# klasmodin/quflow

Measured on AMD Instinct MI355X. Metric: isospectral timesteps/sec at N=1024 (1 GPU) + ensemble steps/sec at 1/2/4/8 GPUs, higher is better.
Workload: dtype f64

## Files before the change

include/quflow_hip.h:

```cpp
#ifndef QUFLOW_HIP_H
#define QUFLOW_HIP_H

#ifdef __cplusplus
extern "C" {
#endif

#define QF_OK 0
#define QF_ERR_INVALID 1
#define QF_ERR_NO_DEVICE 2
#define QF_ERR_HIP 3
#define QF_ERR_STATE 4
#define QF_ERR_CALLBACK 5
#define QF_ERR_UNSUPPORTED 6
#define QF_ERR_NONFINITE 7
#define QF_ERR_NOCONVERGE 8

#define QF_VERSION 100

typedef struct qf_ctx qf_ctx;

int qf_version(void);
const char *qf_last_error(void);
int qf_device_count(void);

// ... 156 lines not shown
#define QF_BUF_W 0
#define QF_BUF_DW 1
#define QF_BUF_WHALF 2
#define QF_BUF_PHALF 3
#define QF_BUF_PW 4
int qf_download_buffer(qf_ctx *ctx, int which, void *host);
int qf_debug_guard_check(long long *allocations, long long *damaged, char *first, int n);
int qf_debug_modulus(qf_ctx *ctx, int n, const double *er_host, const double *ei_host, double *out_modulus_host,
                     double *out_sqrt_host);
int qf_zgemm(qf_ctx *ctx, const void *A_host, const void *B_host, void *C_host);
int qf_commutator(qf_ctx *ctx, const void *W_host, const void *P_host, void *C_host, int skewherm);
int qf_zgemm_i8(qf_ctx *ctx, const void *A_host, const void *B_host, void *C_host);
int qf_fixedpoint_products(qf_ctx *ctx, const void *Phalf_host, const void *Whalf_host, const void *W_host,
                           const void *dW_old_host, int variant, void *dW_new_host, void *Whalf_new_host,
                           double *rowsum_host);

int qf_c64_laplacian_table(qf_ctx *ctx, int bc, float *lap_host);
int qf_c64_solve_poisson(qf_ctx *ctx, const void *W_host, void *P_host, int skewh);
int qf_c64_solve_tridiagonal(qf_ctx *ctx, const float *lap_host, const void *W_host, void *P_host, int skewh);
int qf_c64_laplace(qf_ctx *ctx, const void *P_host, void *W_host);
int qf_c64_upload_W(qf_ctx *ctx, const void *W_host);
int qf_c64_download_W(qf_ctx *ctx, void *W_host);
int qf_c64_isomp(qf_ctx *ctx, double dt, int steps, double tol, int minit, int maxit, int compsum, int reinitialize,
                 qf_isomp_stats *stats_out);
int qf_c64_isomp_continue(qf_ctx *ctx, double dt, int steps, double tol, int minit, int maxit, int compsum, int reinitialize,
                          qf_isomp_stats *stats_out);
int qf_c64_diagnostics(qf_ctx *ctx, double *energy_euler, double *enstrophy);
int qf_cgemm(qf_ctx *ctx, const void *A_host, const void *B_host, void *C_host);
int qf_c64_fixedpoint_products(qf_ctx *ctx, const void *Phalf_host, const void *Whalf_host, const void *W_host,
                               const void *dW_old_host, void *dW_new_host, void *Whalf_new_host, double *rowsum_host);
// ... 16 lines not shown
```

quflow_amd/_lib.py:

```python
import ctypes
import os

_HERE = os.path.dirname(os.path.abspath(__file__))
LIB_PATH = os.environ.get("QUFLOW_HIP_LIB") or os.path.join(_HERE, "libquflow_hip.so")

QF_OK = 0
QF_ERR_NONFINITE = 7
QF_ERR_NOCONVERGE = 8
ERR_NAMES = {1: "QF_ERR_INVALID", 2: "QF_ERR_NO_DEVICE", 3: "QF_ERR_HIP", 4: "QF_ERR_STATE", 5: "QF_ERR_CALLBACK",
             6: "QF_ERR_UNSUPPORTED", 7: "QF_ERR_NONFINITE", 8: "QF_ERR_NOCONVERGE"}

KERNEL_IDS = {"poisson": 0, "gemm1": 1, "gemm2": 2, "norm": 3, "update": 4, "slice": 5}
ERK_METHODS = {"euler": 0, "heun": 1, "rk4": 2}
BUFFER_IDS = {"W": 0, "dW": 1, "Whalf": 2, "Phalf": 3, "PW": 4}


class QuflowHipError(RuntimeError):
    pass


HAMILTONIAN_CB = ctypes.CFUNCTYPE(ctypes.c_int, ctypes.c_void_p, ctypes.c_void_p, ctypes.c_void_p, ctypes.c_double)
FORCING_CB = ctypes.CFUNCTYPE(ctypes.c_int, ctypes.c_void_p, ctypes.c_void_p, ctypes.c_void_p, ctypes.c_void_p, ctypes.c_double)
STRANG_CB = ctypes.CFUNCTYPE(ctypes.c_int, ctypes.c_void_p, ctypes.c_double, ctypes.c_void_p)
CALLBACK_CB = ctypes.CFUNCTYPE(ctypes.c_int, ctypes.c_void_p, ctypes.c_void_p, ctypes.c_void_p)
# ... 134 lines not shown
    "qf_profile_reset": (ctypes.c_int, [_vp]),
    "qf_profile_read": (ctypes.c_int, [_vp, ctypes.c_int, ctypes.POINTER(ctypes.c_longlong), _dp]),
    "qf_plan_describe": (ctypes.c_int, [_vp, ctypes.c_char_p, ctypes.c_int]),
    "qf_device_info": (ctypes.c_int, [ctypes.c_int, ctypes.c_char_p, ctypes.c_int]),
    "qf_debug_modulus": (ctypes.c_int, [_vp, ctypes.c_int, _dp, _dp, _dp, _dp]),
    "qf_profile_stride": (ctypes.c_int, [_vp, ctypes.c_int]),
    "qf_profile_seen": (ctypes.c_int, [_vp, ctypes.c_int, ctypes.POINTER(ctypes.c_longlong)]),
    "qf_timer_start": (ctypes.c_int, [_vp]),
    "qf_timer_stop": (ctypes.c_int, [_vp, _dp]),
    "qf_download_buffer": (ctypes.c_int, [_vp, ctypes.c_int, _vp]),
    "qf_debug_guard_check": (ctypes.c_int, [ctypes.POINTER(ctypes.c_longlong), ctypes.POINTER(ctypes.c_longlong), ctypes.c_char_p, ctypes.c_int]),
    "qf_zgemm": (ctypes.c_int, [_vp, _vp, _vp, _vp]),
    "qf_commutator": (ctypes.c_int, [_vp, _vp, _vp, _vp, ctypes.c_int]),
    "qf_zgemm_i8": (ctypes.c_int, [_vp, _vp, _vp, _vp]),
    "qf_fixedpoint_products": (ctypes.c_int, [_vp, _vp, _vp, _vp, _vp, ctypes.c_int, _vp, _vp, _vp]),
    "qf_c64_laplacian_table": (ctypes.c_int, [_vp, ctypes.c_int, _vp]),
    "qf_c64_solve_poisson": (ctypes.c_int, [_vp, _vp, _vp, ctypes.c_int]),
    "qf_c64_laplace": (ctypes.c_int, [_vp, _vp, _vp]),
    "qf_c64_solve_tridiagonal": (ctypes.c_int, [_vp, _vp, _vp, _vp, ctypes.c_int]),
    "qf_c64_upload_W": (ctypes.c_int, [_vp, _vp]),
    "qf_c64_download_W": (ctypes.c_int, [_vp, _vp]),
    "qf_c64_isomp": (ctypes.c_int, [_vp, ctypes.c_double, ctypes.c_int, ctypes.c_double, ctypes.c_int,
                                    ctypes.c_int, ctypes.c_int, ctypes.c_int, ctypes.POINTER(IsompStats)]),
    "qf_c64_isomp_continue": (ctypes.c_int, [_vp, ctypes.c_double, ctypes.c_int, ctypes.c_double, ctypes.c_int,
                                             ctypes.c_int, ctypes.c_int, ctypes.c_int, ctypes.POINTER(IsompStats)]),
    "qf_c64_diagnostics": (ctypes.c_int, [_vp, _dp, _dp]),
    "qf_cgemm": (ctypes.c_int, [_vp, _vp, _vp, _vp]),
    "qf_c64_fixedpoint_products": (ctypes.c_int, [_vp, _vp, _vp, _vp, _vp, _vp, _vp, _vp]),
    "qf_c64_fixedpoint_products_tri": (ctypes.c_int, [_vp, _vp, _vp, _vp, _vp, _vp, _vp, _vp]),
}
# ... 50 lines not shown
```

quflow_amd/csrc/api_context.hip:

```cpp
#include <cmath>
#include <cstdarg>
#include <cstdio>
#include <cstdlib>
#include <cstring>
#include <limits>
#include <chrono>

#include "qf_api.h"

static thread_local char g_err[512] = "";

void qf_set_error(const char *fmt, ...)
{
    va_list ap;
    va_start(ap, fmt);
    vsnprintf(g_err, sizeof(g_err), fmt, ap);
    va_end(ap);
}

extern "C" {

int qf_version(void) { return QF_VERSION; }

int qf_device_info(int device, char *buf, int n)
// ... 101 lines not shown
        if (g[0] == 'i' && strstr(g, "x65")) ctx->oz_digits2 = 5;
        if (g[0] == 'i' && strchr(g, 'h')) ctx->gemm_i8_hybrid = true;
        if (g[0] == 'i' && strchr(g, 'f') && !ctx->gemm_i8_hybrid) ctx->gemm_i8_first = true;
        if (g[0] == 'a') {
            ctx->gemm_i8_allowed = true;
            ctx->oz_digits = 6;
            ctx->oz_digits2 = 5;
            ctx->gemm_i8_min_n = 1024;
        }
    }
    if (const char *g = getenv("QUFLOW_HIP_GEMM2")) ctx->gemm_tri_allowed = !(g[0] == 'f');
    if (const char *g = getenv("QUFLOW_HIP_FUSED")) ctx->fused_allowed = !(g[0] == '0');
    if (const char *g = getenv("QUFLOW_HIP_I8_MIN_N")) ctx->gemm_i8_min_n = atoi(g);
    if (const char *g = getenv("QUFLOW_HIP_TRI_MIN_N")) ctx->gemm_tri_min_n = atoi(g);
    if (const char *g = getenv("QUFLOW_HIP_DEFER")) ctx->defer_allowed = !(g[0] == '0');
    if (getenv("QUFLOW_HIP_DEBUG"))
        if (const char *g = getenv("QUFLOW_HIP_DEBUG_DROP_FLAG")) ctx->debug_drop = atoi(g);
    if (const char *g = getenv("QUFLOW_HIP_FACTOR_CACHE_MB")) ctx->factor_budget_bytes = (size_t)(atoi(g) > 0 ? atoi(g) : 1) << 20;
    const size_t NN = (size_t)N * N;
    const size_t mbytes = NN * sizeof(cplx);
    int rc = QF_OK;
    auto fail = [&](int code) {
        qf_ctx_destroy(ctx);
        return code;
    };
#define QF_CREATE_HIP(call)                                                                   \
    do {                                                                                      \
        hipError_t _e = (call);                                                               \
        if (_e != hipSuccess) {                                                               \
            qf_set_error("%s failed: %s", #call, hipGetErrorString(_e));                     \
// ... 45 lines not shown
    *out = ctx;
    return QF_OK;
}

int qf_ctx_destroy(qf_ctx *ctx)
{
    if (!ctx) return QF_OK;
    (void)hipSetDevice(ctx->device);
    if (ctx->stream) (void)hipStreamSynchronize(ctx->stream);
    void *ptrs[] = {ctx->W, ctx->dW[0], ctx->dW[1], ctx->Whalf, ctx->Phalf, ctx->PW, ctx->kahan_c, ctx->stage,
                    ctx->lap, ctx->lap_user, ctx->poisson.tab, ctx->ham.tab, ctx->ham_offset, ctx->forcing_f0, ctx->stoch.basis, ctx->stoch.omega,
                    ctx->stoch.stage, ctx->stoch.sigma, ctx->rowpart, ctx->rowsum,
                    ctx->t32_partial, ctx->t32_arrive, ctx->W2, ctx->Whalf2, ctx->ns_inv, ctx->ns_tmp, ctx->multi_rowpart, ctx->scalars, ctx->sk_partial, ctx->sk_flags, ctx->basis, ctx->sh_stage, ctx->sh_omega, ctx->slab};
    for (void *p : ptrs)
        if (p) (void)hipFree(p);
    void *sht[] = {ctx->sht.omega, ctx->sht.tab, ctx->sht.col, ctx->sht.At, ctx->sht.tw, ctx->sht.f, ctx->sht.H, ctx->sht.Q};
    for (void *p : sht)
        if (p) (void)hipFree(p);
    void *eigh[] = {ctx->eigh.H, ctx->eigh.G, ctx->eigh.V, ctx->eigh.ray, ctx->eigh.sig, ctx->eigh.perm, ctx->eigh.word};
    for (void *p : eigh)
        if (p) (void)hipFree(p);
    void *geom[] = {ctx->geom.R[0], ctx->geom.R[1], ctx->geom.grad};
    for (void *p : geom)
        if (p) (void)hipFree(p);
    for (hipEvent_t e : ctx->geom.ev)
        if (e) (void)hipEventDestroy(e);
    for (cplx *p : ctx->multi)
        if (p) (void)hipFree(p);
    for (cplx *p : ctx->stack)
        if (p) (void)hipFree(p);
// ... 221 lines not shown
```

quflow_amd/csrc/api_isomp.hip:

```cpp
#include <cmath>
#include <cstdarg>
#include <cstdio>
#include <cstdlib>
#include <cstring>
#include <limits>
#include <chrono>
#include <type_traits>
#include <utility>

#include "qf_api.h"

namespace {

#ifndef QF_RUN_AHEAD
#define QF_RUN_AHEAD 3
#endif

template <class S> constexpr bool is_c64 = std::is_same<S, qf_c64>::value;

template <class S> S *ws(qf_ctx *ctx)
{
    if constexpr (is_c64<S>) return ctx->c64;
    else return ctx;
}
// ... 910 lines not shown
            return QF_ERR_INVALID;
        }
        QF_TRY(tri32_alloc(ctx));
    }
    const int N = ctx->N;
    const size_t bytes = (size_t)N * N * sizeof(cplx);
    QF_HIP(hipMemcpyAsync(ctx->Phalf, Phalf_host, bytes, hipMemcpyHostToDevice, ctx->stream));
    QF_HIP(hipMemcpyAsync(ctx->Whalf, Whalf_host, bytes, hipMemcpyHostToDevice, ctx->stream));
    QF_HIP(hipMemcpyAsync(ctx->stage, W_host, bytes, hipMemcpyHostToDevice, ctx->stream));
    QF_HIP(hipMemcpyAsync(ctx->dW[0], dW_old_host, bytes, hipMemcpyHostToDevice, ctx->stream));
    QF_TRY(qf_launch_zgemm(ctx, ctx->Phalf, ctx->Whalf, ctx->PW, nullptr));
    qf_epilogue ep = epilogue_of(ctx, false);
    ep.W = ctx->stage;
    const bool saved = ctx->gemm_tri, saved32 = ctx->gemm_tri32;
    const int s_min = ctx->sk_min_units, s_epi = ctx->sk_epi_units, s_so = ctx->tri32_split, s_sd = ctx->tri32_split_diag;
    ctx->gemm_tri = (variant == 1);
    ctx->gemm_tri32 = (variant == 2);
    if (variant == 1) {
        if ((variant_arg >> 8) & 0xff) ctx->sk_min_units = (variant_arg >> 8) & 0xff;
        if ((variant_arg >> 16) & 0xff) ctx->sk_epi_units = ((variant_arg >> 16) & 0xff) - 64;
    } else if (variant == 2) {
        const int so = (variant_arg >> 8) & 15, sd = (variant_arg >> 12) & 15;
        if (so == 1 || so == 2 || so == 4) ctx->tri32_split = so;
        if (sd == 1 || sd == 2 || sd == 4) ctx->tri32_split_diag = sd;
    }
    int rc = qf_launch_zgemm(ctx, ctx->PW, ctx->Phalf, nullptr, &ep);
    ctx->gemm_tri = saved;
    ctx->gemm_tri32 = saved32;
    ctx->sk_min_units = s_min;
    ctx->sk_epi_units = s_epi;
    ctx->tri32_split = s_so;
    ctx->tri32_split_diag = s_sd;
    QF_TRY(rc);
    QF_TRY(qf_launch_sum_rowpart(ctx, ctx->rowpart, variant == 1 ? ctx->N / 64 : variant == 2 ? (ctx->N + 31) / 32 : ctx->rowpart_tiles, ctx->rowsum));
    QF_HIP(hipMemcpyAsync(dW_new_host, ctx->dW[1], bytes, hipMemcpyDeviceToHost, ctx->stream));
    QF_HIP(hipMemcpyAsync(Whalf_new_host, ctx->Whalf, bytes, hipMemcpyDeviceToHost, ctx->stream));
    QF_HIP(hipMemcpyAsync(rowsum_host, ctx->rowsum, (size_t)N * sizeof(double), hipMemcpyDeviceToHost, ctx->stream));
    QF_HIP(hipStreamSynchronize(ctx->stream));
    return QF_OK;
}


int qf_oz_alloc(qf_ctx *ctx)
{
    for (int q = 0; q < 4; ++q) {
// ... 43 lines not shown
```

quflow_amd/csrc/qf_internal.h:

```cpp
#pragma once

#include <hip/hip_runtime.h>

#include <atomic>
#include <cstdarg>
#include <cstdio>
#include <map>
#include <mutex>
#include <string>
#include <vector>

#include "../../include/quflow_hip.h"

typedef double2 cplx;

hipError_t qf_guard_malloc(void **p, size_t bytes);
hipError_t qf_guard_free(void *p);
#define hipMalloc(p, n) qf_guard_malloc((void **)(p), (n))
#define hipFree(p) qf_guard_free((void *)(p))

void qf_set_error(const char *fmt, ...);
struct qf_ctx;
inline void qf_plan_note(qf_ctx *ctx, unsigned long long key, const char *fmt, ...) __attribute__((format(printf, 3, 4)));

#define QF_HIP(call)                                                                   \
// ... 349 lines not shown
    int gemm_tri_min_n = 960;
    bool gemm_tri32 = false;
    int tri32_split = 2, tri32_split_diag = 1;
    cplx *t32_partial = nullptr;
    unsigned *t32_arrive = nullptr;
    bool defer_allowed = true;
    bool defer = false;
    int num_cus = 0;
    cplx *sk_partial = nullptr;
    unsigned *sk_flags = nullptr;
    int sk_slots = 0;
    unsigned sk_epoch = 0;
    int sk_epi_units = 0;
    int sk_epi_units_fused = 2;
    int sk_min_units = 8;
    int debug_drop = 0;
    bool needs_reset = false;

    qf_c64 *c64 = nullptr;

    int profile_mask = 0;
    std::vector<qf_event_pair> events_busy;
    std::vector<qf_event_pair> events_free;
    int profile_stride = 1;
    struct plan_slot {
        unsigned long long key = 0;
        char text[384] = {0};
    } plan[QF_KERNEL_COUNT];
    int plan_role = -1;
    long long prof_seen[QF_KERNEL_COUNT] = {0};
// ... 67 lines not shown
    qf_host_record *rec = nullptr;
    int debug_drop = 0;
};
struct qf_streamk {
    cplx *partial = nullptr;
    unsigned *flags = nullptr;
    unsigned epoch = 0;
    int *fault = nullptr;
    unsigned *ticket = nullptr;
    int n_tiles = 0;
    qf_dev_state *state_rw = nullptr;
    qf_host_record *rec = nullptr;
    unsigned spin_limit = 1u << 22;
    int debug_drop = 0;
    int slots = 0;
};
struct qf_tri32 {
    cplx *partial = nullptr;
    unsigned *arrive = nullptr;
    int split = 1;
    int split_diag = 1;
    unsigned *ticket = nullptr;
    int n_tiles = 0;
    qf_dev_state *state_rw = nullptr;
    qf_host_record *rec = nullptr;
    int debug_drop = 0;
    int deferred = 0;
};
int qf_gemm_tiles_n(int N);
int qf_launch_zgemm_tri32(qf_ctx *ctx, const cplx *A, const cplx *B, const qf_epilogue *ep, qf_guard guard = qf_guard());
int qf_launch_zgemm_tri(qf_ctx *ctx, const cplx *A, const cplx *B, const qf_epilogue *ep, qf_guard guard = qf_guard());
int qf_launch_zgemm(qf_ctx *ctx, const cplx *A, const cplx *B, cplx *C, const qf_epilogue *ep,
                    qf_guard guard = qf_guard());

int qf_launch_basis(qf_ctx *ctx, double *basis_dev);
__host__ __device__ inline long long qf_slab_prefix(int N, int Nmax, int m)
{
    const long long a = m, n = N, k = Nmax;
    return a * n * k - (n + k) * (a * (a - 1) / 2) + (a - 1) * a * (2 * a - 1) / 6;
}
int qf_slab_plan(int N, int Nmax, long long slab_bytes, std::vector<int> &first, long long *max_bytes);
int qf_launch_shr2mat(qf_ctx *ctx, int Nmax, const double *omega_dev, cplx *W_dev);
int qf_launch_band_basis(qf_ctx *ctx, int Nmax, double *band_dev);
int qf_launch_band_shr2mat(qf_ctx *ctx, int Nmax, const double *band_dev, const double *omega_dev, cplx *stage, cplx *W_dev);
int qf_launch_mat2shr(qf_ctx *ctx, int Nmax, const cplx *W_dev, double *omega_dev);
int qf_launch_shc2mat(qf_ctx *ctx, const double *omega_dev, cplx *W_dev);
// ... 73 lines not shown
```

quflow_amd/csrc/zgemm.hip:

```cpp
#include "qf_internal.h"
#include "qf_step_end.h"

#include <cstring>

typedef double v4d __attribute__((ext_vector_type(4)));

#ifdef QF_STAMP
__device__ unsigned long long *qf_stamp_buf = nullptr;
#define QF_STAMP_SLOTS 80
#ifdef QF_STAMP_LIGHT
#define QF_STAMP_AT(slot_)
#define QF_STAMP_PH(kt_, ph_)
__device__ unsigned long long *qf_phase_buf = nullptr;
#else
#define QF_STAMP_AT(slot_)                                                              \
    if (qf_stamp_buf && lane == 0 && (slot_) < QF_STAMP_SLOTS)                          \
        qf_stamp_buf[((size_t)blockIdx.x * (T / 64) + wave) * QF_STAMP_SLOTS + (slot_)] = __builtin_amdgcn_s_memtime();
__device__ unsigned long long *qf_phase_buf = nullptr;
#define QF_STAMP_PH(kt_, ph_)                                                           \
    if (qf_phase_buf && tid == 0 && (kt_) >= 20 && (kt_) < 28)                          \
        qf_phase_buf[((size_t)blockIdx.x * 8 + ((kt_) - 20)) * 5 + (ph_)] = __builtin_amdgcn_s_memtime();
#endif
__device__ unsigned long long *qf_tri_buf = nullptr;
#define QF_TRI_STAMP(seg_, k_)                                                          \
// ... 592 lines not shown
            if (tid == 0) {
                unsigned old = 0u;
                if (!((ep.debug_drop & 2) && lid == 0)) old = __hip_atomic_fetch_add(ep.ticket, 1u, __ATOMIC_RELAXED, __HIP_MEMORY_SCOPE_AGENT);
                *last_flag = (old == (unsigned)(ep.n_tiles - 1)) ? 1u : 0u;
            }
            __syncthreads();
            if (*last_flag != 0u)
                qf_fused_step_end(N, tiles_n, ep.rowpart, ep.ticket, ep.state_rw, ep.rec, guard.iter, tid, rs + WN * BM + 2);
        }
    }
    QF_STAMP_AT(KT + 2)
}

constexpr size_t TRI_SMEM_BYTES = 2 * 64 * 65 * sizeof(cplx) + 4 * 64 * sizeof(double) + 64;

__global__ __launch_bounds__(256) void k_zgemm_tri(int N, int nt, int U, int E, const cplx *__restrict__ A,
                                                    const cplx *__restrict__ B, qf_epilogue ep, qf_guard guard,
                                                    qf_streamk sk)
{
    constexpr int BM = 64, BN = 64, WM = 2, WN = 2;
    constexpr bool EPI = true, EXACT = true, FAST = true;
    using SM = tile_smem<BM, BN, true>;
    constexpr int T = WM * WN * 64;
    constexpr int WTM = BM / WM, WTN = BN / WN;
    constexpr int MT = WTM / 16, NT = WTN / 16;
    constexpr int A_STRIDE = SM::A_STRIDE, B_STRIDE = SM::B_STRIDE;
    constexpr int A_PER = (BM * BK) / T, B_PER = (BN * BK) / T;
    constexpr int A_ROWS_PER = T / BK, B_ROWS_PER = T / BN;
    constexpr int A3_STRIDE = SM::A3_STRIDE, B3_STRIDE = SM::B3_STRIDE;
    constexpr int TS = BN + 1;
    constexpr int TT_BYTES = BM * TS * (int)sizeof(cplx);
    static_assert((size_t)2 * TT_BYTES + (WN * BM + WM * BN) * sizeof(double) + 16 <= TRI_SMEM_BYTES, "epilogue scratch exceeds the LDS request");
    static_assert(TRI_SMEM_BYTES >= SM::main_bytes, "K-loop buffers exceed the LDS request");
    typedef unsigned v4u __attribute__((ext_vector_type(4)));
    constexpr int SG_MFMA = 0x008, SG_VMEM_RD = 0x020, SG_DS_WR = 0x200;

    extern __shared__ __attribute__((aligned(16))) unsigned char smem_raw[];

    const int tid = threadIdx.x;
    const int lane = tid & 63, wave = tid >> 6;
    const int wm = wave / WN, wn = wave % WN;
    const int r16_c = lane & 15, q4_c = lane >> 4;
    const int G = gridDim.x;
    const int c = xcd_remap(blockIdx.x, G);
    const int KTN = N / BK;
    const int S = KTN + E;
    int u = (int)((long long)c * U / G);
    const int u_end = (int)((long long)(c + 1) * U / G);
    const cplx zero = make_double2(0.0, 0.0);

    const unsigned char *lds_fa[2] = {
        smem_raw + (size_t)(q4_c * A_STRIDE + wm * WTM + (r16_c ^ q4_c)) * sizeof(cplx),
        smem_raw + (size_t)(q4_c * A_STRIDE + wm * WTM + (r16_c ^ q4_c ^ 4)) * sizeof(cplx)};
    const unsigned char *lds_fb = smem_raw + SM::B_OFFSET + (size_t)(q4_c * B_STRIDE + wn * WTN + r16_c) * sizeof(cplx);
    unsigned char *lds_sa = smem_raw + (size_t)((tid % BK) * A_STRIDE + ((tid / BK) ^ (tid % BK & 7))) * sizeof(cplx);
    const unsigned char *lds_fa3[2] = {
        smem_raw + SM::A3_OFFSET + (size_t)(q4_c * A3_STRIDE + wm * WTM + 2 * (r16_c ^ q4_c)) * sizeof(double),
        smem_raw + SM::A3_OFFSET + (size_t)(q4_c * A3_STRIDE + wm * WTM + 2 * (r16_c ^ q4_c ^ 4)) * sizeof(double)};
    const unsigned char *lds_fb3 = smem_raw + SM::B3_OFFSET + (size_t)(q4_c * B3_STRIDE + wn * WTN + 2 * r16_c) * sizeof(double);
    unsigned char *lds_sa3 = smem_raw + SM::A3_OFFSET + (size_t)((tid % BK) * A3_STRIDE + 2 * ((tid / BK) ^ (tid % BK & 7))) * sizeof(double);
    const int b_jA = ((tid % 32) / 16) * 32 + (tid % 16);
    unsigned char *lds_sb3 = smem_raw + SM::B3_OFFSET + (size_t)((tid / 32) * B3_STRIDE + 32 * ((tid % 32) / 16) + 2 * (tid % 16)) * sizeof(double);
    unsigned char *lds_sb = smem_raw + SM::B_OFFSET + (size_t)((tid / 32) * B_STRIDE + b_jA) * sizeof(cplx);
// ... 6 lines not shown
    const unsigned p_voff = (unsigned)(tid * sizeof(cplx));
    const unsigned char *a_row = nullptr, *b_col = nullptr;
    const size_t a_pass = 0, b_pass = 0, b_ktile = 0;
    const unsigned a_voff = 0, b_voff = 0;
    const int kt_off = 0;
    const int i0 = 0, j0 = 0;

    cplx e_c[MT][NT][4], e_t[MT][NT][4], e_w[MT][NT][4], e_old[MT][NT][4];
    v4d accR[MT][NT], accI[MT][NT], accS[MT][NT];
    cplx ra[2][A_PER], rb[2][B_PER];
    cplx fa[2][MT], fb[2][NT];
    double fas[2][MT], fbs[2][NT];
#pragma unroll
    for (int r = 0; r < A_PER; ++r) ra[1][r] = rb[1][r] = zero;

#define QF_TRI_KOF(p_) ((p_) <= 0 ? 0 : ((p_) <= E + 1 ? 1 : ((p_) - E > KTN ? KTN : (int)((p_) - E))))
#define QF_TRI_NEXT(u_, found_, t_, k0_, KT_, tm_, tn_)                                \
    {                                                                                  \
        found_ = false;                                                                \
        while (!(found_) && (u_) < u_end) {                                            \
            t_ = (int)((u_) / S);                                                      \
            const int pa_ = (u_) - (t_) * S;                                           \
            int pb_ = u_end - (t_) * S;                                                \
            if (pb_ > S) pb_ = S;                                                      \
            const int klo_ = QF_TRI_KOF(pa_), khi_ = QF_TRI_KOF(pb_);                  \
            u_ = (t_) * S + pb_;                                                       \
            if (klo_ < khi_) {                                                         \
                found_ = true;                                                         \
                k0_ = klo_;                                                            \
                KT_ = khi_ - klo_;                                                     \
                int rem_ = (t_);                                                       \
                tm_ = 0;                                                               \
                while (rem_ >= nt - (tm_)) { rem_ -= nt - (tm_); ++(tm_); }            \
                tn_ = (tm_) + rem_;                                                    \
            }                                                                          \
        }                                                                              \
    }
#define QF_TRI_START_LOADS(k0_, KT_, tm_, tn_)                                         \
    {                                                                                  \
        const int kt_of_segment_ = (KT_);                                              \
        fa_soff0 = (unsigned)(((size_t)(tm_) * BM * N + (size_t)(k0_) * BK) * sizeof(cplx)); \
        fb_soff0 = (unsigned)(((size_t)(k0_) * BK * N + (size_t)(tn_) * BN) * sizeof(cplx)); \
        {                                                                              \
            const int KT = kt_of_segment_;        \
            QF_LOAD_TILE(0, 0)                                                         \
            if (KT > 1) { QF_LOAD_TILE(1, 1) }                                         \
        }                                                                              \
    }
    int seg = 0;
    (void)seg;
// ... 87 lines not shown
                QF_EPI_COMM
            }
            QF_EPI_FETCH(e_w, ep_W, false)
            QF_EPI_FETCH(e_old, ep_dW_old, false)
            double tre[MT][NT][4], tim[MT][NT][4];
#pragma unroll
            for (int mi = 0; mi < MT; ++mi)
#pragma unroll
                for (int ni = 0; ni < NT; ++ni)
#pragma unroll
                    for (int reg = 0; reg < 4; ++reg) {
                        tre[mi][ni][reg] = accR[mi][ni][reg] - accI[mi][ni][reg];
                        tim[mi][ni][reg] = (accS[mi][ni][reg] - accR[mi][ni][reg]) - accI[mi][ni][reg];
                    }
            if (KT < KTN) {
                const int tile_org = t * S, tile_end = tile_org + S;
                const int c_first = c + 1;
                int c_last = c;
                while (c_last + 1 < G && (int)((long long)(c_last + 1) * U / G) < tile_end) ++c_last;
#define QF_TRI_HAS_PIECE(c2_)                                                          \
    (QF_TRI_KOF((int)((long long)(c2_) * U / G) - tile_org) <                          \
     QF_TRI_KOF(((int)(((long long)(c2_) + 1) * U / G) < tile_end ? (int)(((long long)(c2_) + 1) * U / G) : tile_end) - tile_org))
                for (int c2 = c_last; c2 >= c_first; --c2) {
                    const int slot2 = c2;
                    if (!QF_TRI_HAS_PIECE(c2)) continue;
                    if (tid == 0) {
                        unsigned spins = 0;
                        while (__hip_atomic_load(sk.flags + slot2, __ATOMIC_RELAXED, __HIP_MEMORY_SCOPE_AGENT) != sk.epoch) {
                            __builtin_amdgcn_s_sleep(QF_POLL_SLEEP);
                            if (++spins > sk.spin_limit) {
                                *sk.fault = 1;
                                break;
                            }
                        }
                    }
                    asm volatile("s_barrier" ::: "memory");
                    const unsigned soff = (unsigned)((size_t)slot2 * (BM * BN) * sizeof(cplx));
// ... 133 lines not shown
            }
        }
        QF_TRI_STAMP(seg, 3)
        ++seg;
        have = have_next;
        t = n_t;
        k0 = n_k0;
        KT = n_KT;
        tm = n_tm;
        tn = n_tn;
        asm volatile("s_waitcnt lgkmcnt(0)\n\ts_barrier" ::: "memory");
    }
    if (run_finale)
        qf_fused_step_end(N, nt, ep.rowpart, sk.ticket, sk.state_rw, sk.rec, guard.iter, tid, reinterpret_cast<double *>(smem_raw));
#undef QF_TRI_NEXT
#undef QF_TRI_KOF
#undef QF_TRI_HAS_PIECE
#undef QF_TRI_START_LOADS
}

template <bool EXACT>
__global__ __launch_bounds__(256) void k_zgemm_tri32(int N, int nt, const cplx *__restrict__ A, const cplx *__restrict__ B,
                                                      qf_epilogue ep, qf_guard guard, qf_tri32 sx)
{
    if (!qf_guard_iter(guard)) return;
    constexpr int BM = 32, BN = 32, WM = 2, WN = 2;
    constexpr bool EPI = true, FAST = false;
    using SM = tile_smem<BM, BN, false>;
    constexpr int T = WM * WN * 64;
    constexpr int WTM = BM / WM, WTN = BN / WN;
    constexpr int MT = WTM / 16, NT = WTN / 16;
// ... 360 lines not shown
        if (exact) return launch2<BM, BN, WM, WN, true, true>(ctx, A, B, C, *ep, guard);
        return launch2<BM, BN, WM, WN, true, false>(ctx, A, B, C, *ep, guard);
    }
    if (exact) return launch2<BM, BN, WM, WN, false, true>(ctx, A, B, C, none, guard);
    return launch2<BM, BN, WM, WN, false, false>(ctx, A, B, C, none, guard);
}

}

int qf_gemm_tiles_n(int N)
{
    gemm_cfg c = pick_gemm(N);
    return (N + c.BN - 1) / c.BN;
}

int qf_launch_zgemm_tri(qf_ctx *ctx, const cplx *A, const cplx *B, const qf_epilogue *ep, qf_guard guard)
{
    const int N = ctx->N;
    if (!ep || N % 64 != 0 || !ctx->sk_partial || ctx->num_cus < 1) {
        qf_set_error("qf_launch_zgemm_tri: not available for this context (N=%d)", N);
        return QF_ERR_STATE;
    }
    static qf_smem_attr attr;
    QF_TRY(qf_smem_attr_set(attr, (const void *)k_zgemm_tri, ctx->device, TRI_SMEM_BYTES));
    const int nt = N / 64;
    int E = ep->fused ? ctx->sk_epi_units_fused : ctx->sk_epi_units;
    if (E < -8) E = -8;
    const long long units = (long long)nt * (nt + 1) / 2 * (N / BK + E);
    if (units > 0x7fffffffLL) {
        qf_set_error("qf_launch_zgemm_tri: N=%d is too large for the stream-K partition", N);
        return QF_ERR_INVALID;
    }
    long long grid_ll = units / (ctx->sk_min_units > 0 ? ctx->sk_min_units : 1);
    if (grid_ll > ctx->num_cus) grid_ll = ctx->num_cus;
    if (grid_ll < 1) grid_ll = 1;
    const int grid = (int)grid_ll;
    qf_streamk sk;
    const int slots = ctx->sk_slots > 0 ? ctx->sk_slots : ctx->num_cus;
    sk.slots = slots;
    sk.partial = ctx->sk_partial;
    sk.flags = ctx->sk_flags;
    sk.epoch = ++ctx->sk_epoch;
    sk.fault = &ctx->host_rec->fault;
    sk.ticket = ctx->sk_flags + slots;
    sk.n_tiles = nt * (nt + 1) / 2;
    sk.state_rw = ctx->state;
    sk.rec = ctx->host_rec;
    if (ctx->debug_drop == 1 || (ctx->debug_drop == 2 && ep->fused)) {
        sk.debug_drop = ctx->debug_drop;
        sk.spin_limit = 1u << 14;
        ctx->debug_drop = 0;
    }
    qf_plan_note(ctx, 0x2000000ull | (unsigned long long)(grid << 8 | (E & 0x3f) << 1 | (ep->fused ? 1 : 0)),
                 "{\"kernel\": \"k_zgemm_tri\", \"arithmetic\": \"fp64 3M, v_mfma_f64_16x16x4_f64\", \"tile\": [64, 64], \"tiles\": %d, "
                 "\"tile_share\": %.6f, \"workgroups\": %d, \"threads\": 256, \"partition\": \"stream-K over (tile, K-tile) units, "
                 "contiguous ranges, epilogue weight E = %d K-tiles\", \"step_end\": \"%s\"}",
                 sk.n_tiles, (double)sk.n_tiles / ((double)nt * nt), grid, E, ep->fused ? "fused (last finisher decides)" : "two-kernel");
    hipLaunchKernelGGL(k_zgemm_tri, dim3(grid), dim3(256), TRI_SMEM_BYTES, ctx->stream, N, nt, (int)units, E, A, B, *ep, guard, sk);
    QF_HIP(hipGetLastError());
    return QF_OK;
}

int qf_launch_zgemm_tri32(qf_ctx *ctx, const cplx *A, const cplx *B, const qf_epilogue *ep, qf_guard guard)
{
    const int N = ctx->N;
    if (!ep || N < 64 || !ctx->t32_partial || !ctx->t32_arrive) {
        qf_set_error("qf_launch_zgemm_tri32: not available for this context (N=%d)", N);
        return QF_ERR_STATE;
    }
    const int nt = (N + 31) / 32;
    qf_tri32 sx;
    sx.partial = ctx->t32_partial;
    sx.arrive = ctx->t32_arrive;
// ... 36 lines not shown
```

Before: 2701.

## Drive triangular stream-K partition from precomputed per-workgroup boundary table

Replaces the in-kernel uniform stream-K range arithmetic in the triangular ZGEMM with a per-workgroup boundary table built on the host, cached per configuration and uploaded to device memory. Adds an optional 'classes' partition mode that uses a cost model (publish, finish and lead weights, minimum head size) to balance ranges. The default rule still selects uniform mode, so the main change on the default path is simpler per-unit indexing in the kernel plus a table read. This adds a host-side table build, a device allocation on first use, and extra global loads of the boundaries in the fixup loop.

```diff
diff --git a/include/quflow_hip.h b/include/quflow_hip.h
--- a/include/quflow_hip.h
+++ b/include/quflow_hip.h
@@ -194,6 +194,7 @@
 int qf_fixedpoint_products(qf_ctx *ctx, const void *Phalf_host, const void *Whalf_host, const void *W_host,
                            const void *dW_old_host, int variant, void *dW_new_host, void *Whalf_new_host,
                            double *rowsum_host);
+int qf_tri_partition(int N, int G, int min_units, int mode, int E, int *out_bounds);
 
 int qf_c64_laplacian_table(qf_ctx *ctx, int bc, float *lap_host);
 int qf_c64_solve_poisson(qf_ctx *ctx, const void *W_host, void *P_host, int skewh);
diff --git a/quflow_amd/_lib.py b/quflow_amd/_lib.py
--- a/quflow_amd/_lib.py
+++ b/quflow_amd/_lib.py
@@ -172,6 +172,7 @@
     "qf_commutator": (ctypes.c_int, [_vp, _vp, _vp, _vp, ctypes.c_int]),
     "qf_zgemm_i8": (ctypes.c_int, [_vp, _vp, _vp, _vp]),
     "qf_fixedpoint_products": (ctypes.c_int, [_vp, _vp, _vp, _vp, _vp, ctypes.c_int, _vp, _vp, _vp]),
+    "qf_tri_partition": (ctypes.c_int, [ctypes.c_int] * 5 + [ctypes.POINTER(ctypes.c_int)]),
     "qf_c64_laplacian_table": (ctypes.c_int, [_vp, ctypes.c_int, _vp]),
     "qf_c64_solve_poisson": (ctypes.c_int, [_vp, _vp, _vp, ctypes.c_int]),
     "qf_c64_laplace": (ctypes.c_int, [_vp, _vp, _vp]),
diff --git a/quflow_amd/csrc/api_context.hip b/quflow_amd/csrc/api_context.hip
--- a/quflow_amd/csrc/api_context.hip
+++ b/quflow_amd/csrc/api_context.hip
@@ -139,6 +139,8 @@
     if (const char *g = getenv("QUFLOW_HIP_I8_MIN_N")) ctx->gemm_i8_min_n = atoi(g);
     if (const char *g = getenv("QUFLOW_HIP_TRI_MIN_N")) ctx->gemm_tri_min_n = atoi(g);
     if (const char *g = getenv("QUFLOW_HIP_DEFER")) ctx->defer_allowed = !(g[0] == '0');
+    if (const char *g = getenv("QUFLOW_HIP_TRI_PARTITION")) ctx->tri_partition = (g[0] == 'c') ? QF_TRI_MODE_CLASSES : QF_TRI_MODE_UNIFORM;
+    qf_tri_weights_parse(getenv("QUFLOW_HIP_TRI_WEIGHTS"), ctx->tri_weights);
     if (getenv("QUFLOW_HIP_DEBUG"))
         if (const char *g = getenv("QUFLOW_HIP_DEBUG_DROP_FLAG")) ctx->debug_drop = atoi(g);
     if (const char *g = getenv("QUFLOW_HIP_FACTOR_CACHE_MB")) ctx->factor_budget_bytes = (size_t)(atoi(g) > 0 ? atoi(g) : 1) << 20;
@@ -214,6 +216,7 @@
                     ctx->t32_partial, ctx->t32_arrive, ctx->W2, ctx->Whalf2, ctx->ns_inv, ctx->ns_tmp, ctx->multi_rowpart, ctx->scalars, ctx->sk_partial, ctx->sk_flags, ctx->basis, ctx->sh_stage, ctx->sh_omega, ctx->slab};
     for (void *p : ptrs)
         if (p) (void)hipFree(p);
+    qf_tri_tables_free(ctx);
     void *sht[] = {ctx->sht.omega, ctx->sht.tab, ctx->sht.col, ctx->sht.At, ctx->sht.tw, ctx->sht.f, ctx->sht.H, ctx->sht.Q};
     for (void *p : sht)
         if (p) (void)hipFree(p);
diff --git a/quflow_amd/csrc/api_isomp.hip b/quflow_amd/csrc/api_isomp.hip
--- a/quflow_amd/csrc/api_isomp.hip
+++ b/quflow_amd/csrc/api_isomp.hip
@@ -948,11 +948,13 @@
     ep.W = ctx->stage;
     const bool saved = ctx->gemm_tri, saved32 = ctx->gemm_tri32;
     const int s_min = ctx->sk_min_units, s_epi = ctx->sk_epi_units, s_so = ctx->tri32_split, s_sd = ctx->tri32_split_diag;
+    const int s_part = ctx->tri_partition;
     ctx->gemm_tri = (variant == 1);
     ctx->gemm_tri32 = (variant == 2);
     if (variant == 1) {
         if ((variant_arg >> 8) & 0xff) ctx->sk_min_units = (variant_arg >> 8) & 0xff;
         if ((variant_arg >> 16) & 0xff) ctx->sk_epi_units = ((variant_arg >> 16) & 0xff) - 64;
+        ctx->tri_partition = ((variant_arg >> 24) & 1) ? QF_TRI_MODE_CLASSES : QF_TRI_MODE_UNIFORM;
     } else if (variant == 2) {
         const int so = (variant_arg >> 8) & 15, sd = (variant_arg >> 12) & 15;
         if (so == 1 || so == 2 || so == 4) ctx->tri32_split = so;
@@ -963,6 +965,7 @@
     ctx->gemm_tri32 = saved32;
     ctx->sk_min_units = s_min;
     ctx->sk_epi_units = s_epi;
+    ctx->tri_partition = s_part;
     ctx->tri32_split = s_so;
     ctx->tri32_split_diag = s_sd;
     QF_TRY(rc);
diff --git a/quflow_amd/csrc/qf_internal.h b/quflow_amd/csrc/qf_internal.h
--- a/quflow_amd/csrc/qf_internal.h
+++ b/quflow_amd/csrc/qf_internal.h
@@ -9,6 +9,7 @@
 #include <mutex>
 #include <string>
 #include <vector>
+#include "tri_partition.h"
 
 #include "../../include/quflow_hip.h"
 
@@ -388,6 +389,16 @@
     int sk_epi_units = 0;
     int sk_epi_units_fused = 2;
     int sk_min_units = 8;
+    int tri_partition = QF_TRI_MODE_RULE;
+    qf_tri_weights tri_weights;
+    struct tri_table {
+        int N = 0, G = 0, min_units = 0, mode = 0, E = 0;
+        qf_tri_weights w;
+        int used = 0;
+        std::vector<int> host;
+        int *dev = nullptr;
+    };
+    std::vector<tri_table *> tri_tables;
     int debug_drop = 0;
     bool needs_reset = false;
 
@@ -485,6 +496,7 @@
     unsigned spin_limit = 1u << 22;
     int debug_drop = 0;
     int slots = 0;
+    const int *bound = nullptr;
 };
 struct qf_tri32 {
     cplx *partial = nullptr;
@@ -501,6 +513,7 @@
 int qf_gemm_tiles_n(int N);
 int qf_launch_zgemm_tri32(qf_ctx *ctx, const cplx *A, const cplx *B, const qf_epilogue *ep, qf_guard guard = qf_guard());
 int qf_launch_zgemm_tri(qf_ctx *ctx, const cplx *A, const cplx *B, const qf_epilogue *ep, qf_guard guard = qf_guard());
+void qf_tri_tables_free(qf_ctx *ctx);
 int qf_launch_zgemm(qf_ctx *ctx, const cplx *A, const cplx *B, cplx *C, const qf_epilogue *ep,
                     qf_guard guard = qf_guard());
 
diff --git a/quflow_amd/csrc/tri_partition.h b/quflow_amd/csrc/tri_partition.h
--- /dev/null
+++ b/quflow_amd/csrc/tri_partition.h
@@ -0,0 +1,119 @@
+#pragma once
+#include <cstdio>
+#include <vector>
+
+#define QF_TRI_MODE_RULE (-1)
+#define QF_TRI_MODE_UNIFORM 0
+#define QF_TRI_MODE_CLASSES 1
+
+struct qf_tri_weights {
+    int w_pub = 26;
+    int w_fin = 90;
+    int w_lead = 16;
+    int h_min = 8;
+};
+
+inline int qf_tri_mode_rule(int N, int cus) { (void)N; (void)cus; return QF_TRI_MODE_UNIFORM; }
+
+inline void qf_tri_weights_parse(const char *text, qf_tri_weights &w)
+{
+    if (text) sscanf(text, "%d,%d,%d,%d", &w.w_pub, &w.w_fin, &w.w_lead, &w.h_min);
+    if (w.w_pub < 0) w.w_pub = 0;
+    if (w.w_fin < 0) w.w_fin = 0;
+    if (w.h_min < 1) w.h_min = 1;
+}
+
+inline int qf_tri_ktn(int N) { return N / 16; }
+inline int qf_tri_tiles(int N) { return (N / 64) * (N / 64 + 1) / 2; }
+
+inline int qf_tri_grid(int N, int cus, int min_units, int E)
+{
+    const int S = qf_tri_ktn(N) + E;
+    if (S < 1) return 0;
+    long long g = (long long)qf_tri_tiles(N) * S / (min_units > 0 ? min_units : 1);
+    if (g > cus) g = cus;
+    if (g < 1) g = 1;
+    return (int)g;
+}
+
+inline int qf_tri_kof(int p, int E, int KTN) { return p <= 0 ? 0 : (p <= E + 1 ? 1 : (p - E > KTN ? KTN : p - E)); }
+
+inline void qf_tri_table_uniform(int N, int G, int E, std::vector<int> &bound)
+{
+    const int KTN = qf_tri_ktn(N), S = KTN + E;
+    const long long U = (long long)qf_tri_tiles(N) * S;
+    bound.assign((size_t)G + 1, 0);
+    for (int c = 0; c <= G; ++c) {
+        const long long pos = (long long)c * U / G;
+        const long long t = pos / S;
+        bound[(size_t)c] = (int)(t * KTN + qf_tri_kof((int)(pos - t * S), E, KTN));
+    }
+}
+
+inline long long qf_tri_range_time(int u, int e, int KTN, const qf_tri_weights &w)
+{
+    if (e <= u) return 0;
+    const int heads = (e + KTN - 1) / KTN - (u + KTN - 1) / KTN;
+    long long t = 16LL * (e - u) + (u % KTN ? w.w_pub : 0) + (long long)heads * w.w_fin;
+    if (heads == 0) t += w.w_fin + w.w_lead;
+    return t;
+}
+
+inline bool qf_tri_table_classes(int N, int G, int min_units, const qf_tri_weights &w, std::vector<int> &bound)
+{
+    const int KTN = qf_tri_ktn(N);
+    const long long total_ll = (long long)qf_tri_tiles(N) * KTN;
+    if (min_units < 1) min_units = 1;
+    if (G < 1 || total_ll > 0x7fffffffLL || (long long)G * min_units > total_ll) return false;
+    const int total = (int)total_ll;
+    auto end_ok = [&](int u, int e) {
+        const int ke = e % KTN;
+        return ke == 0 || ke >= w.h_min || e - ke < u;
+    };
+    std::vector<int> b((size_t)G + 1);
+    const long long lo = (16LL * total + (long long)qf_tri_tiles(N) * w.w_fin) / G;
+    const long long hi = lo + 32LL * KTN + 2LL * (w.w_pub + w.w_fin + w.w_lead) + 16LL * w.h_min;
+    for (long long T = lo; T <= hi; ++T) {
+        int u = 0;
+        bool ok = true;
+        b[0] = 0;
+        for (int c = 0; c < G && ok; ++c) {
+            const int cap = total - min_units * (G - 1 - c);
+            int e;
+            if (c == G - 1) {
+                e = total;
+                ok = end_ok(u, e) && qf_tri_range_time(u, e, KTN, w) <= T;
+            } else {
+                const int first_head = (u + KTN - 1) / KTN * KTN;
+                e = -1;
+                if (first_head < cap && qf_tri_range_time(u, first_head + 1, KTN, w) <= T) {
+                    int a = first_head + 1, z = cap;
+                    while (a < z) {
+                        const int m = a + (z - a + 1) / 2;
+                        if (qf_tri_range_time(u, m, KTN, w) <= T) a = m;
+                        else z = m - 1;
+                    }
+                    e = a;
+                    if (!end_ok(u, e)) e -= e % KTN;
+                }
+                if (e <= first_head) {
+                    int a = u, z = first_head < cap ? first_head : cap;
+                    while (a < z) {
+                        const int m = a + (z - a + 1) / 2;
+                        if (qf_tri_range_time(u, m, KTN, w) <= T) a = m;
+                        else z = m - 1;
+                    }
+                    e = a;
+                }
+                ok = e - u >= min_units && end_ok(u, e);
+            }
+            b[(size_t)c + 1] = e;
+            u = e;
+        }
+        if (ok) {
+            bound = b;
+            return true;
+        }
+    }
+    return false;
+}
diff --git a/quflow_amd/csrc/zgemm.hip b/quflow_amd/csrc/zgemm.hip
--- a/quflow_amd/csrc/zgemm.hip
+++ b/quflow_amd/csrc/zgemm.hip
@@ -630,7 +630,7 @@
 
 constexpr size_t TRI_SMEM_BYTES = 2 * 64 * 65 * sizeof(cplx) + 4 * 64 * sizeof(double) + 64;
 
-__global__ __launch_bounds__(256) void k_zgemm_tri(int N, int nt, int U, int E, const cplx *__restrict__ A,
+__global__ __launch_bounds__(256) void k_zgemm_tri(int N, int nt, const cplx *__restrict__ A,
                                                     const cplx *__restrict__ B, qf_epilogue ep, qf_guard guard,
                                                     qf_streamk sk)
 {
@@ -660,9 +660,10 @@
     const int G = gridDim.x;
     const int c = xcd_remap(blockIdx.x, G);
     const int KTN = N / BK;
-    const int S = KTN + E;
-    int u = (int)((long long)c * U / G);
-    const int u_end = (int)((long long)(c + 1) * U / G);
+    typedef const __attribute__((address_space(4))) int *bound_ptr;
+    const bound_ptr bound = (bound_ptr)(unsigned long long)sk.bound;
+    int u = bound[c];
+    const int u_end = bound[c + 1];
     const cplx zero = make_double2(0.0, 0.0);
 
     const unsigned char *lds_fa[2] = {
@@ -699,26 +700,20 @@
 #pragma unroll
     for (int r = 0; r < A_PER; ++r) ra[1][r] = rb[1][r] = zero;
 
-#define QF_TRI_KOF(p_) ((p_) <= 0 ? 0 : ((p_) <= E + 1 ? 1 : ((p_) - E > KTN ? KTN : (int)((p_) - E))))
 #define QF_TRI_NEXT(u_, found_, t_, k0_, KT_, tm_, tn_)                                \
     {                                                                                  \
-        found_ = false;                                                                \
-        while (!(found_) && (u_) < u_end) {                                            \
-            t_ = (int)((u_) / S);                                                      \
-            const int pa_ = (u_) - (t_) * S;                                           \
-            int pb_ = u_end - (t_) * S;                                                \
-            if (pb_ > S) pb_ = S;                                                      \
-            const int klo_ = QF_TRI_KOF(pa_), khi_ = QF_TRI_KOF(pb_);                  \
-            u_ = (t_) * S + pb_;                                                       \
-            if (klo_ < khi_) {                                                         \
-                found_ = true;                                                         \
-                k0_ = klo_;                                                            \
-                KT_ = khi_ - klo_;                                                     \
-                int rem_ = (t_);                                                       \
-                tm_ = 0;                                                               \
-                while (rem_ >= nt - (tm_)) { rem_ -= nt - (tm_); ++(tm_); }            \
-                tn_ = (tm_) + rem_;                                                    \
-            }                                                                          \
+        found_ = (u_) < u_end;                                                         \
+        if (found_) {                                                                  \
+            t_ = (u_) / KTN;                                                           \
+            k0_ = (u_) - (t_) * KTN;                                                   \
+            int khi_ = u_end - (t_) * KTN;                                             \
+            if (khi_ > KTN) khi_ = KTN;                                                \
+            KT_ = khi_ - (k0_);                                                        \
+            u_ = (t_) * KTN + khi_;                                                    \
+            int rem_ = (t_);                                                           \
+            tm_ = 0;                                                                   \
+            while (rem_ >= nt - (tm_)) { rem_ -= nt - (tm_); ++(tm_); }                \
+            tn_ = (tm_) + rem_;                                                        \
         }                                                                              \
     }
 #define QF_TRI_START_LOADS(k0_, KT_, tm_, tn_)                                         \
@@ -836,13 +831,11 @@
                         tim[mi][ni][reg] = (accS[mi][ni][reg] - accR[mi][ni][reg]) - accI[mi][ni][reg];
                     }
             if (KT < KTN) {
-                const int tile_org = t * S, tile_end = tile_org + S;
+                const int tile_end = (t + 1) * KTN;
                 const int c_first = c + 1;
                 int c_last = c;
-                while (c_last + 1 < G && (int)((long long)(c_last + 1) * U / G) < tile_end) ++c_last;
-#define QF_TRI_HAS_PIECE(c2_)                                                          \
-    (QF_TRI_KOF((int)((long long)(c2_) * U / G) - tile_org) <                          \
-     QF_TRI_KOF(((int)(((long long)(c2_) + 1) * U / G) < tile_end ? (int)(((long long)(c2_) + 1) * U / G) : tile_end) - tile_org))
+                while (c_last + 1 < G && bound[c_last + 1] < tile_end) ++c_last;
+#define QF_TRI_HAS_PIECE(c2_) (bound[c2_] < bound[(c2_) + 1])
                 for (int c2 = c_last; c2 >= c_first; --c2) {
                     const int slot2 = c2;
                     if (!QF_TRI_HAS_PIECE(c2)) continue;
@@ -1006,7 +999,6 @@
     if (run_finale)
         qf_fused_step_end(N, nt, ep.rowpart, sk.ticket, sk.state_rw, sk.rec, guard.iter, tid, reinterpret_cast<double *>(smem_raw));
 #undef QF_TRI_NEXT
-#undef QF_TRI_KOF
 #undef QF_TRI_HAS_PIECE
 #undef QF_TRI_START_LOADS
 }
@@ -1397,6 +1389,62 @@
     return (N + c.BN - 1) / c.BN;
 }
 
+static int tri_table_of(qf_ctx *ctx, int N, int G, int min_units, int mode, int E, const qf_ctx::tri_table **out)
+{
+    const qf_tri_weights &w = ctx->tri_weights;
+    for (const qf_ctx::tri_table *t : ctx->tri_tables)
+        if (t->N == N && t->G == G && t->min_units == min_units && t->mode == mode && t->E == E && t->w.w_pub == w.w_pub &&
+            t->w.w_fin == w.w_fin && t->w.w_lead == w.w_lead && t->w.h_min == w.h_min) {
+            *out = t;
+            return QF_OK;
+        }
+    qf_ctx::tri_table *t = new qf_ctx::tri_table;
+    t->N = N, t->G = G, t->min_units = min_units, t->mode = mode, t->E = E, t->w = w;
+    t->used = QF_TRI_MODE_UNIFORM;
+    if (mode == QF_TRI_MODE_CLASSES && qf_tri_table_classes(N, G, min_units, w, t->host)) t->used = QF_TRI_MODE_CLASSES;
+    else qf_tri_table_uniform(N, G, E, t->host);
+    const size_t bytes = t->host.size() * sizeof(int);
+    hipError_t e = hipMalloc((void **)&t->dev, bytes);
+    if (e == hipSuccess) e = hipMemcpyAsync(t->dev, t->host.data(), bytes, hipMemcpyHostToDevice, ctx->stream);
+    if (e != hipSuccess) {
+        if (t->dev) (void)hipFree(t->dev);
+        delete t;
+        qf_set_error("qf_launch_zgemm_tri: partition table upload failed: %s", hipGetErrorString(e));
+        return QF_ERR_HIP;
+    }
+    ctx->tri_tables.push_back(t);
+    *out = t;
+    return QF_OK;
+}
+
+void qf_tri_tables_free(qf_ctx *ctx)
+{
+    for (qf_ctx::tri_table *t : ctx->tri_tables) {
+        if (t->dev) (void)hipFree(t->dev);
+        delete t;
+    }
+    ctx->tri_tables.clear();
+}
+
+int qf_tri_partition(int N, int G, int min_units, int mode, int E, int *out_bounds)
+{
+    if (N < 64 || N % 64 != 0 || G < 1 || !out_bounds || (mode != QF_TRI_MODE_UNIFORM && mode != QF_TRI_MODE_CLASSES)) {
+        qf_set_error("qf_tri_partition: N a multiple of 64, G >= 1, mode 0 | 1 and a table of G + 1 ints are needed");
+        return -QF_ERR_INVALID;
+    }
+    if (E < -8) E = -8;
+    const long long units = (long long)qf_tri_tiles(N) * (qf_tri_ktn(N) + E);
+    const int grid = qf_tri_grid(N, G, min_units, E);
+    if (grid < 1 || units > 0x7fffffffLL) {
+        qf_set_error("qf_tri_partition: no cost space for N=%d, E=%d (N / 16 + E must be positive, the units fewer than 2^31)", N, E);
+        return -QF_ERR_INVALID;
+    }
+    std::vector<int> b;
+    if (!(mode == QF_TRI_MODE_CLASSES && qf_tri_table_classes(N, grid, min_units, qf_tri_weights(), b))) qf_tri_table_uniform(N, grid, E, b);
+    for (size_t i = 0; i < b.size(); ++i) out_bounds[i] = b[i];
+    return grid;
+}
+
 int qf_launch_zgemm_tri(qf_ctx *ctx, const cplx *A, const cplx *B, const qf_epilogue *ep, qf_guard guard)
 {
     const int N = ctx->N;
@@ -1410,15 +1458,16 @@
     int E = ep->fused ? ctx->sk_epi_units_fused : ctx->sk_epi_units;
     if (E < -8) E = -8;
     const long long units = (long long)nt * (nt + 1) / 2 * (N / BK + E);
-    if (units > 0x7fffffffLL) {
-        qf_set_error("qf_launch_zgemm_tri: N=%d is too large for the stream-K partition", N);
+    const int grid = qf_tri_grid(N, ctx->num_cus, ctx->sk_min_units, E);
+    if (grid < 1 || units > 0x7fffffffLL) {
+        qf_set_error("qf_launch_zgemm_tri: no stream-K partition for N=%d with the epilogue weight %d", N, E);
         return QF_ERR_INVALID;
     }
-    long long grid_ll = units / (ctx->sk_min_units > 0 ? ctx->sk_min_units : 1);
-    if (grid_ll > ctx->num_cus) grid_ll = ctx->num_cus;
-    if (grid_ll < 1) grid_ll = 1;
-    const int grid = (int)grid_ll;
+    const qf_ctx::tri_table *table = nullptr;
+    const int mode = ctx->tri_partition == QF_TRI_MODE_RULE ? qf_tri_mode_rule(N, ctx->num_cus) : ctx->tri_partition;
+    QF_TRY(tri_table_of(ctx, N, grid, ctx->sk_min_units, mode, E, &table));
     qf_streamk sk;
+    sk.bound = table->dev;
     const int slots = ctx->sk_slots > 0 ? ctx->sk_slots : ctx->num_cus;
     sk.slots = slots;
     sk.partial = ctx->sk_partial;
@@ -1434,12 +1483,15 @@
         sk.spin_limit = 1u << 14;
         ctx->debug_drop = 0;
     }
-    qf_plan_note(ctx, 0x2000000ull | (unsigned long long)(grid << 8 | (E & 0x3f) << 1 | (ep->fused ? 1 : 0)),
+    char mode_text[48];
+    if (table->used == QF_TRI_MODE_CLASSES) snprintf(mode_text, sizeof(mode_text), "classes");
+    else snprintf(mode_text, sizeof(mode_text), "uniform(E = %d K-tiles)", E);
+    qf_plan_note(ctx, 0x2000000ull | (unsigned long long)(table->used << 20 | grid << 8 | (E & 0x3f) << 1 | (ep->fused ? 1 : 0)),
                  "{\"kernel\": \"k_zgemm_tri\", \"arithmetic\": \"fp64 3M, v_mfma_f64_16x16x4_f64\", \"tile\": [64, 64], \"tiles\": %d, "
                  "\"tile_share\": %.6f, \"workgroups\": %d, \"threads\": 256, \"partition\": \"stream-K over (tile, K-tile) units, "
-                 "contiguous ranges, epilogue weight E = %d K-tiles\", \"step_end\": \"%s\"}",
-                 sk.n_tiles, (double)sk.n_tiles / ((double)nt * nt), grid, E, ep->fused ? "fused (last finisher decides)" : "two-kernel");
-    hipLaunchKernelGGL(k_zgemm_tri, dim3(grid), dim3(256), TRI_SMEM_BYTES, ctx->stream, N, nt, (int)units, E, A, B, *ep, guard, sk);
+                 "contiguous ranges from a table, %s\", \"step_end\": \"%s\"}",
+                 sk.n_tiles, (double)sk.n_tiles / ((double)nt * nt), grid, mode_text, ep->fused ? "fused (last finisher decides)" : "two-kernel");
+    hipLaunchKernelGGL(k_zgemm_tri, dim3(grid), dim3(256), TRI_SMEM_BYTES, ctx->stream, N, nt, A, B, *ep, guard, sk);
     QF_HIP(hipGetLastError());
     return QF_OK;
 }
```

Result: no change. 2714, median of 6 (+0.5%).
